# SmartTensors/NMFk.jl

Measured on NVIDIA B200. Metric: nmf_restart_iterations_per_sec, higher is better.
Workload: dtype f32

## Files before the change

nmfk.jl_b200/csrc/kl_tiled.cuh:

```cuda
#pragma once
#include <algorithm>
#include <climits>
#include <cmath>
#include <cstdio>
#include <cstdlib>
#include <type_traits>
#include <chrono>
#include <vector>

#include "kl_resident.cuh"
#include "kl_tiled_args.h"

namespace nmfk {

constexpr int kTiledThreads = 256;
constexpr int kTiledStages = 3;

template <typename TX>
struct TiledCfg {
    static constexpr int TCH = sizeof(TX) == 8 ? 16 : 32;
};


template <typename TX, typename TC, int K, bool HASNAN>
// ... 631 lines not shown
        fprintf(stderr, "\n");
        for (auto e : idle) cudaEventDestroy(e);
        idle.clear();
    }
};

#define NMFK_TRY(call)                      \
    do {                                    \
        cudaError_t e__ = (call);           \
        if (e__ != cudaSuccess) {           \
            err = e__;                      \
            goto done;                      \
        }                                   \
    } while (0)

template <typename TX, typename TC>
cudaError_t solve_tiled_t(const SolveArgs& a, cudaStream_t s, int64_t* launches) {
    const int n = a.n, m = a.m, k = a.k, R = a.R;
    const int kt = tiled_template_k(k);
    if (kt < 0) return cudaErrorInvalidValue;
    cudaError_t err = cudaSuccess;
    int sms = 148;
    {
        int dev = 0;
        cudaGetDevice(&dev);
        cudaDeviceGetAttribute(&sms, cudaDevAttrMultiProcessorCount, dev);
    }
    bool use_tc = false;
    if (std::is_same<TX, float>::value && std::is_same<TC, float>::value && a.tiled_tc && !a.has_nan) {
        TiledPassArgs probe{};
        probe.k = k;
        probe.nown = m;
        probe.D = a.Xt;
        use_tc = tc_pass_supported(probe);
        probe.nown = n;
        probe.D = a.X;
        use_tc = use_tc && tc_pass_supported(probe);
    }
    const bool use_td = std::is_same<TX, double>::value && std::is_same<TC, double>::value && a.tiled_tc && !a.has_nan && k >= 4;
    const int ownper = use_tc ? 128 : (use_td ? tiled_dmma_own() : kTiledThreads);
    const int units = use_tc ? (R + tc_pass_group(k) - 1) / tc_pass_group(k) : R;
    const int nblkH = (m + ownper - 1) / ownper;
    const int nblkW = (n + ownper - 1) / ownper;
    constexpr int TCH = TiledCfg<TX>::TCH;
    const double slice_gain = getenv("NMFK_TILED_SLICE_GAIN") ? atof(getenv("NMFK_TILED_SLICE_GAIN")) : 0.05;
    auto slices = [&](int nblk, int nred) {
        const long long target = (use_tc ? 3ll * tc_pass_ctas_per_sm(k) : (use_td ? 3ll : 4ll)) * sms;
        long long S = (target + (long long)nblk * units - 1) / ((long long)nblk * units);
        const long long smax = std::max(1, nred / ((use_tc ? tc_pass_chunk(k) : (use_td ? tiled_dmma_chunk() : TCH)) * 8));
        if (S > smax) S = smax;
        if (S < 1) S = 1;
        auto eff = [&](long long s_) {
            const long long ctas = (long long)nblk * units * s_;
            return (double)ctas / (double)(((ctas + sms - 1) / sms) * sms);
        };
        long long best = S;
        for (long long s2 = S + 1; s2 <= std::min(smax, S + 3); ++s2)
            if (eff(s2) > eff(best) + slice_gain) best = s2;
        return (int)best;
    };
    const int SH = slices(nblkH, n), SW = slices(nblkW, m);
    const int nblkObj = (n + 127) / 128;
    const bool wobj = a.wref.any();

    const ShardComm* sh = a.shard;
    const bool sharded = sh != nullptr;
    PhaseTimer pt;
    pt.on = getenv("NMFK_TILED_TIMING") != nullptr;
    const auto host_t0 = std::chrono::steady_clock::now();
    auto host_ms = [&]() { return std::chrono::duration<double, std::milli>(std::chrono::steady_clock::now() - host_t0).count(); };
    double host_setup_ms = 0.0;
    const int it_begin_report = 0;
    (void)it_begin_report;
    TC* den = nullptr;
    TC* red = nullptr;
    double* obj2 = nullptr;
    TC* partial = nullptr;
    double* objp = nullptr;
    int* d_active = nullptr;
    double* fin_tot = nullptr;
    int* fin_flag = nullptr;
    void* vimg = nullptr;
    int* h_active = nullptr;
    const char* flag_kernel = use_tc && tc2_pass_enabled(k) ? "tc2_pass_kernel or tc_pass_kernel" : "tc_pass_kernel";
    const char* flag_where = "half-update pass or stop-check objective";
    std::vector<UnitState> hst((size_t)R);
    int it = 0;
    bool any_running = false;
    const size_t psz = std::max((size_t)((SH > 1 || sharded) ? (size_t)SH * R * m * kt : 0),
                                (size_t)(SW > 1 ? (size_t)SW * R * n * kt : 0));
    const size_t redsz = sharded ? (size_t)R * m * kt : 0;
    if (sharded && a.normalize == 2) return cudaErrorNotSupported;
    const int wait_hint = getenv("NMFK_TC_WAIT_HINT_NS") ? atoi(getenv("NMFK_TC_WAIT_HINT_NS")) : ((32 << 16) | 64);
    const int qwait = getenv("NMFK_TC_QWAIT_NS") ? atoi(getenv("NMFK_TC_QWAIT_NS")) : 0;
    auto obj_args = [&](int restore, int sel) {
        TiledPassArgs po{};
        po.D = use_td ? a.Xt : a.X;
        po.U = a.W;
        po.V = a.H;
        po.st = a.st;
        po.u_rstride = (long long)n * k;
        po.v_rstride = (long long)k * m;
        po.su_o = 1;
        po.su_a = n;
        po.sv_t = k;
        po.sv_a = 1;
        po.nown = n;
        po.nred = m;
        po.k = k;
        po.R = R;
        po.S = 1;
        po.nblocks = nblkObj;
        po.lambda = a.lambda;
        po.ktmpl = kt;
        po.obj_partials = objp;
        po.obj_weight = a.weight;
        po.obj_restore = restore;
        po.obj_sel = sel;
        po.wait_hint_ns = wait_hint;
        po.qwait_ns = qwait;
        return po;
    };

    NMFK_TRY(scratch_alloc(&den, ((size_t)R * kTiledMaxK + redsz) * sizeof(TC), s));
    if (sharded) red = den + (size_t)R * kTiledMaxK;
    NMFK_TRY(scratch_alloc(&obj2, (size_t)R * 2 * sizeof(double), s));
    if (psz) NMFK_TRY(scratch_alloc(&partial, psz * sizeof(TC), s));
    NMFK_TRY(scratch_alloc(&objp, (size_t)R * nblkObj * 2 * sizeof(double), s));
    NMFK_TRY(scratch_alloc(&d_active, sizeof(int), s));
    NMFK_TRY(scratch_alloc(&fin_tot, (size_t)R * kTiledMaxK * sizeof(double), s));
    NMFK_TRY(scratch_alloc(&fin_flag, (size_t)R * sizeof(int), s));
    if (use_tc) {
        const size_t vb = std::max(tc2_image_bytes(k, R, n), tc2_image_bytes(k, R, m));
        if (vb) NMFK_TRY(scratch_alloc(&vimg, vb, s));
    }
    h_active = pinned_flags();
    if (h_active == nullptr) NMFK_TRY(cudaErrorMemoryAllocation);
    h_active[0] = h_active[1] = 0;
    h_active[1] = 0;
    NMFK_TRY(cudaMemcpyAsync(hst.data(), a.st, (size_t)R * sizeof(UnitState), cudaMemcpyDeviceToHost, s));
    NMFK_TRY(cudaStreamSynchronize(s));
    for (auto& u : hst)
        if (u.stop == 0 && !u.done) {
            any_running = true;
            it = std::max(it, (int)u.it);
        }
    if (any_running) {
        TiledPassArgs ph{}, pw{};
        ph.D = use_td ? a.X : a.Xt;
        ph.Dstep = a.X;
        ph.U = a.H;
        ph.V = a.W;
        ph.den = den;
        ph.partial = (SH > 1 || sharded) ? partial : nullptr;
        ph.st = a.st;
        ph.ximp = a.ximp;
        ph.u_rstride = (long long)k * m;
        ph.v_rstride = (long long)n * k;
        ph.su_o = k;
        ph.su_a = 1;
        ph.sv_t = 1;
        ph.sv_a = n;
        ph.nown = m;
        ph.nred = n;
        ph.k = k;
        ph.R = R;
        ph.S = SH;
        ph.nblocks = nblkH;
        ph.transposed = 1;
        ph.ldimp = n;
        ph.has_nan = a.has_nan;
        ph.lambda = a.lambda;
        ph.ktmpl = kt;
        ph.vimg = vimg;
        ph.wait_hint_ns = wait_hint;
        ph.qwait_ns = qwait;
        pw = ph;
        pw.D = use_td ? a.Xt : a.X;
        pw.Dstep = a.Xt;
        pw.U = a.W;
        pw.V = a.H;
        pw.partial = SW > 1 ? partial : nullptr;
        pw.u_rstride = (long long)n * k;
        pw.v_rstride = (long long)k * m;
        pw.su_o = 1;
        pw.su_a = n;
        pw.sv_t = k;
        pw.sv_a = 1;
        pw.nown = n;
        pw.nred = m;
        pw.S = SW;
        pw.nblocks = nblkW;
        pw.transposed = 0;

        if (a.has_nan && it > 0) {
            dim3 g((n + 127) / 128, R);
            tiled_impute_kernel<TX, TC><<<g, 128, 0, s>>>((const TX*)a.X, n, m, k, (const TC*)a.W, (const TC*)a.H, a.st,
                                                          (TC*)a.ximp);
            NMFK_TRY(cudaGetLastError());
            ++*launches;
        }
        long long* d_trace = nullptr;
        const char* trace_path = use_tc ? getenv("NMFK_TC_TRACE") : nullptr;
// ... 11 lines not shown
                                                                   d_active);
                NMFK_TRY(cudaGetLastError());
                ++*launches;
                NMFK_TRY(cudaMemcpyAsync(h_active, d_active, sizeof(int), cudaMemcpyDeviceToHost, s));
                pt.mark(s, 10);
                NMFK_TRY(cudaStreamSynchronize(s));
                if (a.prof) a.prof->harvest();
                pt.harvest();
                if (h_active[1] != 0) goto done;
                if (*h_active == 0) break;
                need_guard = false;
                pt.mark(s, -1);
            }
            ++it;
            ph.first_iter = pw.first_iter = (it == 1);
            if (!a.Hfixed) {
                tiled_sums_kernel<TC><<<dim3(k, R), 256, 0, s>>>(a.W, (long long)n * k, 1, n, n, a.st, den);
                NMFK_TRY(cudaGetLastError());
                pt.mark(s, 0);
                NMFK_TRY((timed_tiled_pass<TX, TC>(ph, red, s, use_tc, h_active + 1, use_td, a.prof)));
                pt.mark(s, 1);
                *launches += 2 + (SH > 1 || sharded) + (vimg != nullptr);
                if (d_trace != nullptr) {
                    std::vector<long long> ht(3 * 64 * 8);
                    NMFK_TRY(cudaMemcpyAsync(ht.data(), d_trace, ht.size() * sizeof(long long), cudaMemcpyDeviceToHost, s));
                    NMFK_TRY(cudaStreamSynchronize(s));
                    if (FILE* f = fopen(trace_path, "wb")) {
                        fwrite(ht.data(), sizeof(long long), ht.size(), f);
                        fclose(f);
                    }
                    cudaFree(d_trace);
                    d_trace = nullptr;
                    ph.trace = nullptr;
                }
                if (sharded) {
                    NMFK_TRY(sh->allreduce(sh->comm, den, (size_t)R * kTiledMaxK + redsz, sizeof(TC) == 8 ? 1 : 0, s));
                    pt.mark(s, 2);
                    NMFK_TRY((dispatch_tiled_apply<TX, TC>(ph, red, s)));
                    pt.mark(s, 3);
                    ++*launches;
                }
            }
            if (!a.Wfixed) {
                tiled_sums_kernel<TC><<<dim3(k, R), 256, 0, s>>>(a.H, (long long)k * m, k, 1, m, a.st, den);
                NMFK_TRY(cudaGetLastError());
                pt.mark(s, 4);
                NMFK_TRY((timed_tiled_pass<TX, TC>(pw, nullptr, s, use_tc, h_active + 1, use_td, a.prof)));
                pt.mark(s, 5);
                *launches += 2 + (SW > 1) + (vimg != nullptr);
            }
            if (a.has_nan) {
                dim3 g((n + 127) / 128, R);
                tiled_impute_kernel<TX, TC><<<g, 128, 0, s>>>((const TX*)a.X, n, m, k, (const TC*)a.W, (const TC*)a.H,
                                                              a.st, (TC*)a.ximp);
                NMFK_TRY(cudaGetLastError());
                ++*launches;
            }
            if (it % a.check_every == 0) {
                if (use_tc && !wobj) {
                    NMFK_TRY(launch_tc_objective(obj_args(0, 0), h_active + 1, s));
                } else if (use_td && !wobj) {
                    NMFK_TRY(launch_tiled_dmma_objective(obj_args(0, 0), s));
                } else {
                    dim3 g(nblkObj, R);
                    NMFK_TRY((tiled_objective_smem<TX, TC>(k)));
                    tiled_objective_kernel<TX, TC><<<g, 128, (size_t)k * 128 * sizeof(TC), s>>>(
                        (const TX*)a.X, n, m, k, (const TC*)a.W, (const TC*)a.H, a.st, (TC)a.lambda, 0, 1, a.weight, a.wref, objp);
                }
                NMFK_TRY(cudaGetLastError());
                pt.mark(s, 7);
                tiled_objsum_kernel<<<(R + 127) / 128, 128, 0, s>>>(objp, nblkObj, R, obj2);
                NMFK_TRY(cudaGetLastError());
                ++*launches;
                if (sharded) NMFK_TRY(sh->allreduce(sh->comm, obj2, (size_t)R * 2, 1, s));
                pt.mark(s, 8);
                const bool wide_clamp = (long long)n * k >= (1ll << 18) && !a.Wfixed;
                if (wide_clamp) {
                    const long long nk = (long long)n * k;
                    dim3 g((unsigned)std::min<long long>((nk + 2047) / 2048, 4096), R);
                    tiled_clampW_kernel<TC><<<g, 256, 0, s>>>((TC*)a.W, nk, a.st, obj2, a.tol, (TC)a.eps_clamp);
                    NMFK_TRY(cudaGetLastError());
                    ++*launches;
                }
                TiledCheckArgs c{};
                c.W = a.W;
                c.H = a.H;
                c.st = a.st;
                c.canon = a.canon;
                c.partials = obj2;
                c.n = n;
                c.m = m;
                c.k = k;
                c.nblk = 1;
                c.w_clamped = wide_clamp ? 1 : 0;
                c.it = it;
                c.maxbad = a.maxbad;
                c.stopconv = a.stopconv;
                c.tol = a.tol;
                c.tolOF = a.tolOF;
                c.eps_clamp = a.eps_clamp;
                {
                    const size_t csm = (size_t)(m + k) * sizeof(int);
                    if (csm > 48 * 1024)
                        NMFK_TRY(cudaFuncSetAttribute(tiled_check_kernel<TC>, cudaFuncAttributeMaxDynamicSharedMemorySize, (int)csm));
                    tiled_check_kernel<TC><<<R, 256, csm, s>>>(c);
                }
                NMFK_TRY(cudaGetLastError());
                pt.mark(s, 9);
                *launches += 2;
                need_guard = true;
            }
            if (it >= a.maxiter || (a.iter_limit > 0 && it >= a.iter_limit)) need_guard = true;
        }
    }
    {
        pt.mark(s, -1);
        flag_kernel = "tc_pass_kernel";
        flag_where = "post-run objective";
        if (use_tc && !wobj) {
            NMFK_TRY(launch_tc_objective(obj_args(1, 1), h_active + 1, s));
        } else if (use_td && !wobj) {
            NMFK_TRY(launch_tiled_dmma_objective(obj_args(1, 1), s));
        } else {
            dim3 g(nblkObj, R);
            NMFK_TRY((tiled_objective_smem<TX, TC>(k)));
            tiled_objective_kernel<TX, TC><<<g, 128, (size_t)k * 128 * sizeof(TC), s>>>(
                (const TX*)a.X, n, m, k, (const TC*)a.W, (const TC*)a.H, a.st, (TC)a.lambda, 1, 0, a.weight, a.wref, objp);
        }
        NMFK_TRY(cudaGetLastError());
        if (sharded) {
            tiled_objsum_kernel<<<(R + 127) / 128, 128, 0, s>>>(objp, nblkObj, R, obj2);
            NMFK_TRY(cudaGetLastError());
            NMFK_TRY(sh->allreduce(sh->comm, obj2, (size_t)R * 2, 1, s));
            ++*launches;
        }
        const bool wide_finish = a.normalize == 1 && (long long)n * k >= (1ll << 18);
        if (wide_finish) NMFK_TRY(cudaMemsetAsync(fin_flag, 0, (size_t)R * sizeof(int), s));
        tiled_finish_kernel<TC><<<R, 256, 0, s>>>(a.W, a.H, a.st, sharded ? obj2 : objp, n, m, k, sharded ? 1 : nblkObj,
                                                  a.normalize, wide_finish ? fin_tot : nullptr, wide_finish ? fin_flag : nullptr);
        NMFK_TRY(cudaGetLastError());
        if (wide_finish) {
            const long long nk = (long long)n * k;
            dim3 g((unsigned)std::min<long long>((nk + 2047) / 2048, 1024), R);
            tiled_scaleW_kernel<TC><<<g, 256, 0, s>>>((TC*)a.W, n, k, fin_tot, fin_flag);
            NMFK_TRY(cudaGetLastError());
            ++*launches;
        }
        *launches += 2;
        pt.mark(s, 11);
        NMFK_TRY(cudaStreamSynchronize(s));
        if (a.prof) a.prof->harvest();
        pt.harvest();
        if (pt.on) fprintf(stderr, "[nmfk timing] host wall clock: set-up %.1f ms, whole solve %.1f ms\n", host_setup_ms, host_ms());
        pt.report(it, sharded ? sh->rank : 0);
    }
done:
    if (h_active && h_active[1] != 0) err = solve_timeout(a, err, flag_kernel, flag_where, h_active[1]);
    scratch_free(den, s);
    scratch_free(partial, s);
    scratch_free(objp, s);
    scratch_free(obj2, s);
    scratch_free(d_active, s);
    scratch_free(fin_tot, s);
    scratch_free(fin_flag, s);
    scratch_free(vimg, s);
    return err;
}

}
```

nmfk.jl_b200/csrc/kl_tiled_args.h:

```cpp
#pragma once
#include "nmfk_internal.h"

namespace nmfk {

struct TiledPassArgs {
    const void* D;
    void* U;
    const void* V;
    const void* den;
    void* partial;
    const UnitState* st;
    const void* ximp;
    long long u_rstride, v_rstride;
    long long su_o, su_a, sv_t, sv_a;
    int nown, nred, k, R, S, nblocks;
    int transposed;
    int ldimp;
    int has_nan, first_iter;
    double lambda;
    double* obj_partials;
    double obj_weight;
    int obj_restore;
    int obj_sel;
    int wait_hint_ns;
    int qwait_ns;
    long long* trace;
    int ktmpl;
    const void* Dstep;
    void* vimg;
};

bool tc_pass_supported(const TiledPassArgs& a);
int tc_pass_group(int k);
int tc_pass_ctas_per_sm(int k);
int tc_pass_chunk(int k);
cudaError_t launch_tc_pass(const TiledPassArgs& a, int* d_errflag, cudaStream_t s);
bool tc2_pass_enabled(int k);
cudaError_t launch_tc2_pass(const TiledPassArgs& a, int* d_errflag, cudaStream_t s);
size_t tc2_image_bytes(int k, int R, int nred);
void tc2_pass_prepare();
cudaError_t launch_tc_objective(const TiledPassArgs& a, int* d_errflag, cudaStream_t s);

int tiled_dmma_own();
int tiled_dmma_chunk();
cudaError_t launch_tiled_dmma_pass(const TiledPassArgs& a, cudaStream_t s);
cudaError_t launch_tiled_dmma_objective(const TiledPassArgs& a, cudaStream_t s);

}
```

nmfk.jl_b200/csrc/kl_tiled_tc.cu:

```cuda
#include <algorithm>

#include "kl_tiled_args.h"
#include "tc_ptx.cuh"
#include "tc_stage.cuh"

namespace nmfk {
namespace {

constexpr int TC_M = 128;

template <int K8, int N2>
struct TcCfg {
    static constexpr int TS = 64;
    static constexpr int NXS = K8 <= 32 ? 3 : 2;
    static constexpr int NRAW = K8 <= 32 ? 4 : 2;
    static constexpr int NVB = K8 <= 16 ? 4 : (K8 <= 32 ? 3 : 2);
    static constexpr int RPAD = K8 > 24 ? 0 : 4;
    static constexpr int QW = TS / 4;
    static constexpr int SW = 4;
    static constexpr int QW0 = 2 + SW;
    static constexpr int THREADS = (QW0 + QW) * 32;
    static constexpr int TCOLS = 512;
    static constexpr int NCS = QW / 4;
    static constexpr int NST = N2 == 16 ? 2 : 1;
// ... 437 lines not shown
            tc::named_bar_sync(2, TC_QWARPS * 32);
            if (grp == 1)
#pragma unroll
                for (int c = 0; c < NC2; ++c) xch[c * 256 + slot] = acc[0][c];
            tc::named_bar_sync(2, TC_QWARPS * 32);
            if (grp == 0)
#pragma unroll
                for (int c = 0; c < NC2; ++c) acc[0][c] += xch[c * 256 + slot];
        }
#pragma unroll
        for (int i = 0; i < SL; ++i) {
            const int b = 2 * i + grp;
            if (b < nreal && valid) {
                const int r = s_act[b];
                if (a.partial == nullptr) {
                    float* U = Ug + (long long)r * a.u_rstride;
                    const float* den = static_cast<const float*>(a.den) + (long long)r * kTiledMaxK;
#pragma unroll
                    for (int c = 0; c < NC2; ++c) {
                        const int col = hh * NC2 + c;
                        if (col < k) {
                            const long long idx = (long long)o * a.su_o + (long long)col * a.su_a;
                            U[idx] = (U[idx] * acc[i][c]) / den[col];
                        }
                    }
                } else {
                    float* dst = static_cast<float*>(a.partial) + (((long long)slice * a.R + r) * a.nown + o) * a.ktmpl;
#pragma unroll
                    for (int c = 0; c < NC2; ++c) {
                        const int col = hh * NC2 + c;
                        if (col < a.ktmpl) dst[col] = acc[i][c];
                    }
                }
            }
        }
        }
        __syncwarp();
    }
    tc::tc_fence_before_sync();
    __syncthreads();
    if (warp == 0) tc::tmem_dealloc<C::TCOLS>(tbase);
}

template <int K8, int N2, bool OBJ>
cudaError_t launch_tc(const TiledPassArgs& a, int* d_errflag, cudaStream_t s) {
    using C = TcCfg<K8, N2>;
    const int ngroups = (a.R + C::RB - 1) / C::RB;
    const long long grid = (long long)a.S * a.nblocks * ngroups;
    if (grid > 2147483647ll) return cudaErrorInvalidValue;
    cudaError_t e = cudaFuncSetAttribute(tc_pass_kernel<K8, N2, OBJ>, cudaFuncAttributeMaxDynamicSharedMemorySize, (int)C::SMEM);
    if (e != cudaSuccess) return e;
    tc_pass_kernel<K8, N2, OBJ><<<(unsigned)grid, C::THREADS, C::SMEM, s>>>(a, d_errflag);
    return cudaGetLastError();
}

}

int tc_pass_group(int k) {
    if (k <= 8) return TcCfg<8, 16>::RB;
    if (k <= 16) return TcCfg<16, 16>::RB;
    if (k <= 24) return TcCfg<24, 32>::RB;
    if (k <= 32) return TcCfg<32, 32>::RB;
    if (k <= 48) return TcCfg<48, 64>::RB;
    return TcCfg<64, 64>::RB;
}
int tc_pass_ctas_per_sm(int) { return 1; }
int tc_pass_chunk(int) { return 64; }

bool tc_pass_supported(const TiledPassArgs& a) {
    return !a.has_nan && a.k >= 1 && a.k <= kTiledMaxK && (a.nown % 4) == 0 && (reinterpret_cast<uintptr_t>(a.D) % 16) == 0;
}

cudaError_t launch_tc_pass(const TiledPassArgs& a, int* d_errflag, cudaStream_t s) {
    if (tc2_pass_enabled(a.k)) return launch_tc2_pass(a, d_errflag, s);
    if (a.k <= 8) return launch_tc<8, 16, false>(a, d_errflag, s);
    if (a.k <= 16) return launch_tc<16, 16, false>(a, d_errflag, s);
    if (a.k <= 24) return launch_tc<24, 32, false>(a, d_errflag, s);
    if (a.k <= 32) return launch_tc<32, 32, false>(a, d_errflag, s);
    if (a.k <= 48) return launch_tc<48, 64, false>(a, d_errflag, s);
    return launch_tc<64, 64, false>(a, d_errflag, s);
}

cudaError_t launch_tc_objective(const TiledPassArgs& a, int* d_errflag, cudaStream_t s) {
    if (a.k <= 8) return launch_tc<8, 16, true>(a, d_errflag, s);
    if (a.k <= 16) return launch_tc<16, 16, true>(a, d_errflag, s);
    if (a.k <= 24) return launch_tc<24, 32, true>(a, d_errflag, s);
    if (a.k <= 32) return launch_tc<32, 32, true>(a, d_errflag, s);
    if (a.k <= 48) return launch_tc<48, 64, true>(a, d_errflag, s);
    return launch_tc<64, 64, true>(a, d_errflag, s);
}

}
```

nmfk.jl_b200/csrc/kl_tiled_tc2.cu:

```cuda
#include <algorithm>
#include <cstdlib>
#include <mutex>

#include "kl_tiled_args.h"
#include "tc_ptx.cuh"
#include "tc_stage.cuh"
#include "tma.cuh"

namespace nmfk {
namespace {

constexpr int T2_M = 128;

template <int K8>
struct Tc2Cfg {
    static constexpr int N2 = 16;
    static constexpr int TS = 64;
    static constexpr int NXS = 3;
    static constexpr int NVB = 6;
    static constexpr int QW = TS / 4;
    static constexpr int QW0 = 2;
    static constexpr int LW = QW0 + QW;
    static constexpr int THREADS = (LW + 1) * 32;
    static constexpr int TCOLS = 512;
    static constexpr int RB = 4;
    static constexpr int ACOLS = 2 * N2;
    static constexpr int PBASE = 0, QBASE = 2 * TS, ABASE = QBASE + 2 * 2 * TS, UBASE = ABASE + 2 * ACOLS;
    static constexpr int PERB = K8;
    static_assert(UBASE + RB * PERB <= TCOLS, "tensor memory");
    static constexpr uint32_t U1_BYTES = T2_M * K8 * 4;
    static constexpr uint32_t SBO1 = (K8 / 4) * 128;
    static constexpr uint32_t SBO2 = (TS / 4) * 128;
    static constexpr uint32_t B1_BYTES = TS * K8 * 4;
    static constexpr uint32_t B2_BYTES = N2 * TS * 4;
    static constexpr uint32_t V_BYTES = 2 * B1_BYTES + 2 * B2_BYTES;
    static constexpr uint32_t X_BYTES = TS * T2_M * 4;
    static constexpr int XBOX = 32;
    static constexpr size_t SMEM = (size_t)NXS * X_BYTES + (size_t)NVB * V_BYTES + (size_t)RB * U1_BYTES + 32 * 8 + 64;
    static_assert(SMEM <= 232448, "shared memory budget of one CTA");
};

__device__ __forceinline__ unsigned long long pack2f(float lo, float hi) {
    unsigned long long v;
    asm("mov.b64 %0, {%1, %2};" : "=l"(v) : "f"(lo), "f"(hi));
    return v;
}
__device__ __forceinline__ float rcp_approx(float p) {
    float r;
    asm("rcp.approx.ftz.f32 %0, %1;" : "=f"(r) : "f"(p));
    return r;
}

template <int K8>
__global__ void __launch_bounds__(256) tc2_images_kernel(const TiledPassArgs a, int chunks) {
    using C = Tc2Cfg<K8>;
    const int c = blockIdx.x, r = blockIdx.y;
    if (a.st[r].stop != 0) return;
    const float* V = static_cast<const float*>(a.V) + (long long)r * a.v_rstride;
    float4* img = reinterpret_cast<float4*>(static_cast<unsigned char*>(a.vimg) + ((size_t)r * chunks + c) * C::V_BYTES);
    const int t0 = c * C::TS;
    auto val = [&](int t, int col) {
        return (t0 + t < a.nred && col < a.k) ? V[(long long)(t0 + t) * a.sv_t + (long long)col * a.sv_a] : 0.f;
    };
    constexpr int NAB = K8 / 4, NTB = C::TS / 4;
    constexpr int NA = C::TS * NAB, NB = C::N2 * NTB;
    for (int it = threadIdx.x; it < NA + NB; it += blockDim.x) {
        float v[4];
        int hi, lo;
        if (it < NA) {
            const int t = (it & 7) + 8 * (it / (8 * NAB)), ab = (it >> 3) % NAB;
#pragma unroll
            for (int j = 0; j < 4; ++j) v[j] = val(t, ab * 4 + j);
            hi = it;
            lo = it + C::B1_BYTES / 16;
        } else {
            const int ib = it - NA;
            const int col = (ib & 7) + 8 * (ib / (8 * NTB)), tb = (ib >> 3) % NTB;
#pragma unroll
            for (int i = 0; i < 4; ++i) v[i] = val(tb * 4 + i, col);
            hi = 2 * C::B1_BYTES / 16 + ib;
            lo = hi + C::B2_BYTES / 16;
        }
        float h[4], l[4];
#pragma unroll
        for (int j = 0; j < 4; ++j) {
            h[j] = __uint_as_float(__float_as_uint(v[j]) & 0xffffe000u);
            l[j] = v[j] - h[j];
        }
        img[hi] = make_float4(h[0], h[1], h[2], h[3]);
        img[lo] = make_float4(l[0], l[1], l[2], l[3]);
    }
}

template <int K8>
__global__ void __launch_bounds__((Tc2Cfg<K8>::THREADS), 1) tc2_pass_kernel(const TiledPassArgs a, const __grid_constant__ CUtensorMap mX,
                                                                            int* errflag) {
    using C = Tc2Cfg<K8>;
    constexpr int NXS = C::NXS, NVB = C::NVB, TS = C::TS, QWARPS = C::QW, QW0 = C::QW0;
    constexpr int RB = C::RB, N2 = C::N2;
    extern __shared__ __align__(1024) unsigned char smem[];
    float* Xs = reinterpret_cast<float*>(smem);
    unsigned char* Vs = smem + (size_t)NXS * C::X_BYTES;
    unsigned char* Us = Vs + (size_t)NVB * C::V_BYTES;
    uint64_t* bars = reinterpret_cast<uint64_t*>(Us + (size_t)RB * C::U1_BYTES);
    uint64_t* x_full = bars;
    uint64_t* x_empty = x_full + NXS;
    uint64_t* v_full = x_empty + NXS;
    uint64_t* v_empty = v_full + NVB;
    uint64_t* p_full = v_empty + NVB;
    uint64_t* p_empty = p_full + 2;
    uint64_t* q_full = p_empty + 2;
    uint64_t* a_full = q_full + 2;
    uint32_t* tmem_slot = reinterpret_cast<uint32_t*>(bars + 32);
    int* s_act = reinterpret_cast<int*>(tmem_slot + 1);

    const int tid = threadIdx.x, warp = tid >> 5, lane = tid & 31;
    long long* const trc = (a.trace != nullptr && blockIdx.x == 0) ? a.trace : nullptr;
    const int ngroups = (a.R + RB - 1) / RB;
    const int g = blockIdx.x % ngroups;
    const int rest = blockIdx.x / ngroups;
    const int ob = rest % a.nblocks;
    const int slice = rest / a.nblocks;
    const int o0 = ob * T2_M;
    const int k = a.k;
    const int chunks_all = (a.nred + TS - 1) / TS;
    const int t_begin = (int)(((long long)chunks_all * slice) / a.S) * TS;
    const int t_end = min(a.nred, (int)(((long long)chunks_all * (slice + 1)) / a.S) * TS);
    const int nchunks = (t_end - t_begin + TS - 1) / TS;

    if (tid == 0) {
        int nact = 0;
        for (int b = 0; b < RB; ++b) {
            const int r = g * RB + b;
            if (r >= a.R) continue;
            if (a.st[r].stop == 0) s_act[nact++] = r;
        }
        s_act[RB] = nact;
        if (nact & 1) s_act[nact] = s_act[0];
    }
    __syncthreads();
    const int nreal = s_act[RB];
    const int nact = nreal + (nreal & 1);
    if (nreal == 0 || nchunks <= 0) return;
    const int total = nchunks * nact;

    if (warp == 0) tc::tmem_alloc<C::TCOLS>(tmem_slot);
    if (tid == 32) {
        for (int i = 0; i < NXS; ++i) {
// ... 234 lines not shown
                            float q = xv[j] * rcp_approx(__uint_as_float(p[jj]));
                            q = (jh + half * 16 + jj < cnt) ? q : 0.f;
                            const uint32_t h = __float_as_uint(q) & 0xffffe000u;
                            lo[j] = __float_as_uint(q - __uint_as_float(h));
                            p[jj] = h;
                        }
                    }
                    if (prev_slot >= 0) {
                        if (half == 0) {
                            if (warp == QW0) TC_STAMP(0, u, 5);
                            tc::mbar_wait_h(0u, &a_full[grp], (uint32_t)(((u - 2) >> 1) & 1), errflag, 44);
                            tc::tc_fence_after_sync();
                            if (warp == QW0) TC_STAMP(0, u, 6);
                        } else {
                            tc::tmem_wait_ld();
                            drain_add(prev_slot);
                        }
                        drain_load(half);
                    }
                    tc::tmem_st16(qcol + half * 16, p);
                    tc::tmem_st16(qcol + TS + half * 16, lo);
                    if (half == 0 && warp == QW0) TC_STAMP(0, u, 7);
                }
                if (prev_slot >= 0) {
                    tc::tmem_wait_ld();
                    drain_add(prev_slot);
                }
                if (warp == QW0) TC_STAMP(0, u, 3);
                tc::tmem_wait_st();
                tc::tc_fence_before_sync();
                __syncwarp();
                if (lane == 0) tc::mbar_arrive(&q_full[grp]);
                if (warp == QW0) TC_STAMP(0, u, 4);
                prev_slot = b >> 1;
            }
            __syncwarp();
            if (lane == 0) tc::mbar_arrive(&x_empty[s]);
        }
        {
            const int ulast = (nchunks - 1) * nact + (nact - 2 + grp);
            tc::mbar_wait_h(0u, &a_full[grp], (uint32_t)((ulast >> 1) & 1), errflag, 43);
            tc::tc_fence_after_sync();
#pragma unroll
            for (int part = 0; part < 2; ++part) {
                drain_load(part);
                tc::tmem_wait_ld();
                drain_add(prev_slot);
            }
        }
#pragma unroll
        for (int i = 0; i < SL; ++i) {
            const int b = 2 * i + grp;
            if (b < nreal && valid) {
                const int r = s_act[b];
                if (a.partial == nullptr) {
                    float* U = Ug + (long long)r * a.u_rstride;
                    const float* den = static_cast<const float*>(a.den) + (long long)r * kTiledMaxK;
#pragma unroll
                    for (int c = 0; c < NC2; ++c) {
                        const int col = hh * NC2 + c;
                        if (col < k) {
                            const long long idx = (long long)o * a.su_o + (long long)col * a.su_a;
                            U[idx] = (U[idx] * acc[i][c]) / den[col];
                        }
                    }
                } else {
                    float* dst = static_cast<float*>(a.partial) + (((long long)slice * a.R + r) * a.nown + o) * a.ktmpl;
#pragma unroll
                    for (int c = 0; c < NC2; ++c) {
                        const int col = hh * NC2 + c;
                        if (col < a.ktmpl) dst[col] = acc[i][c];
                    }
                }
            }
        }
        __syncwarp();
    }
    tc::tc_fence_before_sync();
    __syncthreads();
    if (warp == 0) tc::tmem_dealloc<C::TCOLS>(tbase);
}

template <int K8>
cudaError_t launch2(const TiledPassArgs& a, int* d_errflag, cudaStream_t s) {
    using C = Tc2Cfg<K8>;
    const int ngroups = (a.R + C::RB - 1) / C::RB;
    const long long grid = (long long)a.S * a.nblocks * ngroups;
    const int chunks = (a.nred + C::TS - 1) / C::TS;
    if (grid > 2147483647ll || a.vimg == nullptr || a.R > 65535) return cudaErrorInvalidValue;
    cudaError_t e = cudaFuncSetAttribute(tc2_pass_kernel<K8>, cudaFuncAttributeMaxDynamicSharedMemorySize, (int)C::SMEM);
    if (e != cudaSuccess) return e;
    struct Cached {
        const void* base;
        int nown, nred;
        CUtensorMap map;
    };
    static std::mutex mu;
    static Cached cache[4];
    static int next = 0;
    CUtensorMap mX;
    {
        std::lock_guard<std::mutex> lock(mu);
        int hit = -1;
        for (int i = 0; i < 4; ++i)
            if (cache[i].base == a.Dstep && cache[i].nown == a.nown && cache[i].nred == a.nred) hit = i;
        if (hit < 0) {
            hit = next;
            next = (next + 1) % 4;
            cache[hit].base = nullptr;
            if (!tma_make_map_f32(&cache[hit].map, a.Dstep, a.nred, a.nown, a.nred, C::XBOX, T2_M, CU_TENSOR_MAP_SWIZZLE_128B))
                return cudaErrorNotSupported;
            cache[hit].base = a.Dstep;
            cache[hit].nown = a.nown;
            cache[hit].nred = a.nred;
        }
        mX = cache[hit].map;
    }
    tc2_images_kernel<K8><<<dim3((unsigned)chunks, (unsigned)a.R), 256, 0, s>>>(a, chunks);
    e = cudaGetLastError();
    if (e != cudaSuccess) return e;
    tc2_pass_kernel<K8><<<(unsigned)grid, C::THREADS, C::SMEM, s>>>(a, mX, d_errflag);
    return cudaGetLastError();
}

}

bool tc2_pass_enabled(int k) {
    static const int gen = [] {
        const char* e = std::getenv("NMFK_TC_GEN");
        return e ? std::atoi(e) : 2;
    }();
    return gen >= 2 && k <= 16 && tma_encode_fn() != nullptr;
}

size_t tc2_image_bytes(int k, int R, int nred) {
    const size_t per = k <= 8 ? Tc2Cfg<8>::V_BYTES : Tc2Cfg<16>::V_BYTES;
    constexpr int TS = Tc2Cfg<16>::TS;
    return tc2_pass_enabled(k) ? (size_t)R * (size_t)((nred + TS - 1) / TS) * per : 0;
}

void tc2_pass_prepare() {
    static bool done = false;
    if (done) return;
    done = true;
    CUtensorMap m;
    float* dummy = nullptr;
    if (cudaMalloc(&dummy, 1 << 20) == cudaSuccess) {
        (void)tma_make_map_f32(&m, dummy, 512, 512, 512, 32, T2_M, CU_TENSOR_MAP_SWIZZLE_128B);
        cudaFree(dummy);
    }
    cudaFuncAttributes fa;
    cudaFuncGetAttributes(&fa, tc2_pass_kernel<8>);
    cudaFuncGetAttributes(&fa, tc2_pass_kernel<16>);
    cudaFuncSetAttribute(tc2_pass_kernel<8>, cudaFuncAttributeMaxDynamicSharedMemorySize, (int)Tc2Cfg<8>::SMEM);
    cudaFuncSetAttribute(tc2_pass_kernel<16>, cudaFuncAttributeMaxDynamicSharedMemorySize, (int)Tc2Cfg<16>::SMEM);
}

cudaError_t launch_tc2_pass(const TiledPassArgs& a, int* d_errflag, cudaStream_t s) {
    if (a.k <= 8) return launch2<8>(a, d_errflag, s);
    return launch2<16>(a, d_errflag, s);
}

}
```

Baseline: 7466.

## Add TMA/tcgen05 pipelined objective kernel for tc2 path

Adds a new warp-specialized objective kernel that uses TMA loads of X, bulk copies of precomputed V images, and split-TF32 tensor-memory MMAs to compute the Frobenius objective, replacing the older tc objective when tc2 is enabled. It reuses the tc2 image kernel in an objective-only mode and factors the tensor map cache into a shared helper. The aim is faster stop-check objective evaluations. The cost is an extra image-building launch per objective and more complex barrier pipelines.

```diff
diff --git a/nmfk.jl_b200/csrc/kl_tiled.cuh b/nmfk.jl_b200/csrc/kl_tiled.cuh
--- a/nmfk.jl_b200/csrc/kl_tiled.cuh
+++ b/nmfk.jl_b200/csrc/kl_tiled.cuh
@@ -737,7 +737,8 @@
     int* fin_flag = nullptr;
     void* vimg = nullptr;
     int* h_active = nullptr;
-    const char* flag_kernel = use_tc && tc2_pass_enabled(k) ? "tc2_pass_kernel or tc_pass_kernel" : "tc_pass_kernel";
+    const bool tc2 = use_tc && tc2_pass_enabled(k);
+    const char* flag_kernel = tc2 ? "tc2_pass_kernel or tc2_objective_kernel" : "tc_pass_kernel";
     const char* flag_where = "half-update pass or stop-check objective";
     std::vector<UnitState> hst((size_t)R);
     int it = 0;
@@ -774,6 +775,8 @@
         po.obj_sel = sel;
         po.wait_hint_ns = wait_hint;
         po.qwait_ns = qwait;
+        po.Dstep = a.Xt;
+        po.vimg = vimg;
         return po;
     };
 
@@ -951,6 +954,7 @@
                     NMFK_TRY(cudaGetLastError());
                     ++*launches;
                 }
+                if (tc2 && !wobj) ++*launches;
                 TiledCheckArgs c{};
                 c.W = a.W;
                 c.H = a.H;
@@ -984,10 +988,11 @@
     }
     {
         pt.mark(s, -1);
-        flag_kernel = "tc_pass_kernel";
+        flag_kernel = tc2 ? "tc2_objective_kernel" : "tc_pass_kernel";
         flag_where = "post-run objective";
         if (use_tc && !wobj) {
             NMFK_TRY(launch_tc_objective(obj_args(1, 1), h_active + 1, s));
+            if (tc2) ++*launches;
         } else if (use_td && !wobj) {
             NMFK_TRY(launch_tiled_dmma_objective(obj_args(1, 1), s));
         } else {
diff --git a/nmfk.jl_b200/csrc/kl_tiled_args.h b/nmfk.jl_b200/csrc/kl_tiled_args.h
--- a/nmfk.jl_b200/csrc/kl_tiled_args.h
+++ b/nmfk.jl_b200/csrc/kl_tiled_args.h
@@ -40,6 +40,7 @@
 size_t tc2_image_bytes(int k, int R, int nred);
 void tc2_pass_prepare();
 cudaError_t launch_tc_objective(const TiledPassArgs& a, int* d_errflag, cudaStream_t s);
+cudaError_t launch_tc2_objective(const TiledPassArgs& a, int* d_errflag, cudaStream_t s);
 
 int tiled_dmma_own();
 int tiled_dmma_chunk();
diff --git a/nmfk.jl_b200/csrc/kl_tiled_tc.cu b/nmfk.jl_b200/csrc/kl_tiled_tc.cu
--- a/nmfk.jl_b200/csrc/kl_tiled_tc.cu
+++ b/nmfk.jl_b200/csrc/kl_tiled_tc.cu
@@ -543,6 +543,7 @@
 }
 
 cudaError_t launch_tc_objective(const TiledPassArgs& a, int* d_errflag, cudaStream_t s) {
+    if (tc2_pass_enabled(a.k) && a.vimg != nullptr && a.Dstep != nullptr) return launch_tc2_objective(a, d_errflag, s);
     if (a.k <= 8) return launch_tc<8, 16, true>(a, d_errflag, s);
     if (a.k <= 16) return launch_tc<16, 16, true>(a, d_errflag, s);
     if (a.k <= 24) return launch_tc<24, 32, true>(a, d_errflag, s);
diff --git a/nmfk.jl_b200/csrc/kl_tiled_tc2.cu b/nmfk.jl_b200/csrc/kl_tiled_tc2.cu
--- a/nmfk.jl_b200/csrc/kl_tiled_tc2.cu
+++ b/nmfk.jl_b200/csrc/kl_tiled_tc2.cu
@@ -51,19 +51,26 @@
     return r;
 }
 
-template <int K8>
+template <bool OBJ>
+__device__ __forceinline__ bool tc2_takes(const TiledPassArgs& a, int r) {
+    const bool stopped = a.st[r].stop != 0;
+    return (OBJ && a.obj_sel == 1) ? (stopped && a.st[r].done == 0) : !stopped;
+}
+
+template <int K8, bool OBJ>
 __global__ void __launch_bounds__(256) tc2_images_kernel(const TiledPassArgs a, int chunks) {
     using C = Tc2Cfg<K8>;
+    constexpr uint32_t IMG = OBJ ? 2 * C::B1_BYTES : C::V_BYTES;
     const int c = blockIdx.x, r = blockIdx.y;
-    if (a.st[r].stop != 0) return;
+    if (!tc2_takes<OBJ>(a, r)) return;
     const float* V = static_cast<const float*>(a.V) + (long long)r * a.v_rstride;
-    float4* img = reinterpret_cast<float4*>(static_cast<unsigned char*>(a.vimg) + ((size_t)r * chunks + c) * C::V_BYTES);
+    float4* img = reinterpret_cast<float4*>(static_cast<unsigned char*>(a.vimg) + ((size_t)r * chunks + c) * IMG);
     const int t0 = c * C::TS;
     auto val = [&](int t, int col) {
         return (t0 + t < a.nred && col < a.k) ? V[(long long)(t0 + t) * a.sv_t + (long long)col * a.sv_a] : 0.f;
     };
     constexpr int NAB = K8 / 4, NTB = C::TS / 4;
-    constexpr int NA = C::TS * NAB, NB = C::N2 * NTB;
+    constexpr int NA = C::TS * NAB, NB = OBJ ? 0 : C::N2 * NTB;
     for (int it = threadIdx.x; it < NA + NB; it += blockDim.x) {
         float v[4];
         int hi, lo;
@@ -464,6 +471,319 @@
 }
 
 template <int K8>
+struct Tc2ObjCfg {
+    using C = Tc2Cfg<K8>;
+    static constexpr int TS = C::TS, RB = C::RB;
+    static constexpr int NXS = 3;
+    static constexpr int NVB = 8;
+    static constexpr int NP = 6;
+    static constexpr int SW0 = 2;
+    static constexpr int NSW = TS / 4;
+    static constexpr int THREADS = (SW0 + NSW) * 32;
+    static constexpr int TCOLS = 512;
+    static constexpr int PBASE = 0, UBASE = NP * TS;
+    static_assert(UBASE + RB * C::PERB <= TCOLS, "tensor memory");
+    static constexpr uint32_t IMG = 2 * C::B1_BYTES;
+    static constexpr int NBARS = 2 * (NXS + NVB + NP);
+    static constexpr size_t SMEM = (size_t)NXS * C::X_BYTES + (size_t)NVB * IMG + (size_t)RB * C::U1_BYTES + NBARS * 8 + 64;
+    static_assert(SMEM <= 232448, "shared memory budget of one CTA");
+};
+
+template <int K8>
+__global__ void __launch_bounds__((Tc2ObjCfg<K8>::THREADS), 1) tc2_objective_kernel(const TiledPassArgs a,
+                                                                                    const __grid_constant__ CUtensorMap mX, int* errflag) {
+    using C = Tc2Cfg<K8>;
+    using O = Tc2ObjCfg<K8>;
+    constexpr int NXS = O::NXS, NVB = O::NVB, NP = O::NP, TS = O::TS, RB = O::RB, SW0 = O::SW0, NSW = O::NSW;
+    extern __shared__ __align__(1024) unsigned char smem[];
+    float* Xs = reinterpret_cast<float*>(smem);
+    unsigned char* Vs = smem + (size_t)NXS * C::X_BYTES;
+    unsigned char* Us = Vs + (size_t)NVB * O::IMG;
+    uint64_t* bars = reinterpret_cast<uint64_t*>(Us + (size_t)RB * C::U1_BYTES);
+    uint64_t* x_full = bars;
+    uint64_t* x_empty = x_full + NXS;
+    uint64_t* v_full = x_empty + NXS;
+    uint64_t* v_empty = v_full + NVB;
+    uint64_t* p_full = v_empty + NVB;
+    uint64_t* p_empty = p_full + NP;
+    uint32_t* tmem_slot = reinterpret_cast<uint32_t*>(bars + O::NBARS);
+    int* s_act = reinterpret_cast<int*>(tmem_slot + 1);
+
+    const int tid = threadIdx.x, warp = tid >> 5, lane = tid & 31;
+    const int ngroups = (a.R + RB - 1) / RB;
+    const int g = blockIdx.x % ngroups;
+    const int ob = blockIdx.x / ngroups;
+    const int o0 = ob * T2_M;
+    const int k = a.k;
+    const int nchunks = (a.nred + TS - 1) / TS;
+
+    if (tid == 0) {
+        int nact = 0;
+        for (int b = 0; b < RB; ++b) {
+            const int r = g * RB + b;
+            if (r < a.R && tc2_takes<true>(a, r)) s_act[nact++] = r;
+        }
+        s_act[RB] = nact;
+    }
+    __syncthreads();
+    const int nact = s_act[RB];
+    if (nact == 0 || nchunks <= 0) return;
+    const int total = nchunks * nact;
+
+    if (warp == 0) tc::tmem_alloc<O::TCOLS>(tmem_slot);
+    if (tid == 32) {
+        for (int i = 0; i < NXS; ++i) {
+            tc::mbar_init(&x_full[i], 1);
+            tc::mbar_init(&x_empty[i], NSW);
+        }
+        for (int i = 0; i < NVB; ++i) {
+            tc::mbar_init(&v_full[i], 1);
+            tc::mbar_init(&v_empty[i], 1);
+        }
+        for (int i = 0; i < NP; ++i) {
+            tc::mbar_init(&p_full[i], 1);
+            tc::mbar_init(&p_empty[i], NSW);
+        }
+        tc::mbar_fence_init();
+    }
+    if (tid == 0) tma_prefetch_map(&mX);
+
+    tc::fence_async_smem();
+    tc::tc_fence_before_sync();
+    __syncthreads();
+    tc::tc_fence_after_sync();
+    const uint32_t tbase = *tmem_slot;
+
+    if (warp >= SW0) {
+        const int lq = warp & 3, cs = (warp - SW0) >> 2;
+        const int ol = lq * 32 + lane;
+        const int o = o0 + ol;
+        const bool valid = o < a.nown;
+        const uint32_t lane_base = tbase + ((uint32_t)(lq * 32) << 16);
+        if (cs < nact) {
+            const float* U = static_cast<const float*>(a.U) + (long long)s_act[cs] * a.u_rstride;
+            const uint32_t col = O::UBASE + cs * C::PERB;
+            unsigned char* img = Us + (size_t)cs * C::U1_BYTES + (ol & 7) * 16 + (ol >> 3) * C::SBO1;
+#pragma unroll
+            for (int c0 = 0; c0 < K8; c0 += 8) {
+                uint32_t hi[8];
+                float lo[8];
+#pragma unroll
+                for (int c = 0; c < 8; ++c) {
+                    const float u = !valid ? 1.f : (c0 + c < k ? U[(long long)o * a.su_o + (long long)(c0 + c) * a.su_a] : 0.f);
+                    hi[c] = __float_as_uint(u) & 0xffffe000u;
+                    lo[c] = u - __uint_as_float(hi[c]);
+                }
+                tc::tmem_st8(lane_base + col + c0, hi);
+                *reinterpret_cast<float4*>(img + (c0 / 4) * TC_LBO) = make_float4(lo[0], lo[1], lo[2], lo[3]);
+                *reinterpret_cast<float4*>(img + (c0 / 4 + 1) * TC_LBO) = make_float4(lo[4], lo[5], lo[6], lo[7]);
+            }
+        }
+        tc::tmem_wait_st();
+    }
+    tc::fence_async_smem();
+    tc::tc_fence_before_sync();
+    __syncthreads();
+    tc::tc_fence_after_sync();
+
+    if (warp == 0) {
+        constexpr uint32_t idP = tc::idesc_tf32(T2_M, TS, 0);
+        const uint64_t d1 = tc::smem_desc(tc::smem_u32(Vs), TC_LBO, C::SBO1);
+        const uint64_t du = tc::smem_desc(tc::smem_u32(Us), TC_LBO, C::SBO1);
+        constexpr uint64_t KSTEP = (2 * TC_LBO) >> 4;
+        int b = 0, vb = 0, pt = 0;
+        for (int u = 0; u < total; ++u) {
+            if (u >= NP) tc::mbar_wait_h(0u, &p_empty[pt], (uint32_t)((u / NP - 1) & 1), errflag, 51);
+            tc::mbar_wait_h(0u, &v_full[vb], (uint32_t)((u / NVB) & 1), errflag, 50);
+            tc::tc_fence_after_sync();
+            const uint32_t d = tbase + O::PBASE + (uint32_t)pt * TS;
+            const uint32_t uh = tbase + O::UBASE + b * C::PERB;
+            const uint64_t al = du + (uint64_t)((b * C::U1_BYTES) >> 4);
+            const uint64_t bh = d1 + (uint64_t)((vb * O::IMG) >> 4), bl = bh + (C::B1_BYTES >> 4);
+            if (tc::elect_one()) {
+#pragma unroll
+                for (int ks = 0; ks < K8 / 8; ++ks) {
+                    tc::mma_tf32_ss(d, al + ks * KSTEP, bh + ks * KSTEP, idP, ks > 0);
+                    tc::mma_tf32_ts(d, uh + ks * 8, bl + ks * KSTEP, idP, 1);
+                    tc::mma_tf32_ts(d, uh + ks * 8, bh + ks * KSTEP, idP, 1);
+                }
+                tc::mma_commit(&p_full[pt]);
+                tc::mma_commit(&v_empty[vb]);
+            }
+            __syncwarp();
+            b = b + 1 == nact ? 0 : b + 1;
+            vb = vb + 1 == NVB ? 0 : vb + 1;
+            pt = pt + 1 == NP ? 0 : pt + 1;
+        }
+        __syncwarp();
+    } else if (warp == 1) {
+        auto load_x = [&](int c, int s) {
+            if (tc::elect_one()) {
+                tc::mbar_arrive_expect_tx(&x_full[s], C::X_BYTES);
+                tma_load_2d(Xs + (size_t)s * TS * T2_M, &mX, c * TS, o0, &x_full[s]);
+                tma_load_2d(Xs + (size_t)s * TS * T2_M + C::XBOX * T2_M, &mX, c * TS + C::XBOX, o0, &x_full[s]);
+            }
+            __syncwarp();
+        };
+        for (int c = 0; c < NXS && c < nchunks; ++c) load_x(c, c);
+        const unsigned char* vimg = static_cast<const unsigned char*>(a.vimg);
+        int c = 0, b = 0, s = 0;
+        int vb = 0, vround = 0;
+        for (int w = 0; w < total; ++w) {
+            if (b == 0 && c >= NXS) {
+                tc::mbar_wait_h(0u, &x_empty[s], (uint32_t)((c / NXS - 1) & 1), errflag, 52);
+                load_x(c, s);
+            }
+            if (vround > 0) tc::mbar_wait_h(0u, &v_empty[vb], (uint32_t)((vround - 1) & 1), errflag, 53);
+            if (tc::elect_one()) {
+                tc::mbar_arrive_expect_tx(&v_full[vb], O::IMG);
+                tc::bulk_g2s(Vs + (size_t)vb * O::IMG, vimg + ((size_t)s_act[b] * nchunks + c) * O::IMG, O::IMG, &v_full[vb]);
+            }
+            __syncwarp();
+            if (++vb == NVB) vb = 0, ++vround;
+            if (++b == nact) {
+                b = 0;
+                ++c;
+                s = s + 1 == NXS ? 0 : s + 1;
+            }
+        }
+        __syncwarp();
+    } else {
+        const int lq = warp & 3, cs = (warp - SW0) >> 2;
+        const int o_loc = lq * 32 + lane;
+        const bool valid = o0 + o_loc < a.nown;
+        const uint32_t lane_base = tbase + ((uint32_t)(lq * 32) << 16);
+        const int j0 = cs * 16;
+        const uint32_t xrow = (uint32_t)((cs >> 1) * C::XBOX * T2_M + o_loc * C::XBOX) * 4;
+        const uint32_t xsw = ((tc::smem_u32(Xs) + xrow) >> 7) & 7;
+        const uint32_t xp0 = (uint32_t)(cs & 1) * 4;
+        double sacc[RB];
+#pragma unroll
+        for (int b = 0; b < RB; ++b) sacc[b] = 0.0;
+        const float lambda = (float)a.lambda;
+        const bool restore = a.obj_restore != 0;
+        auto pull = [&](int u, int t, uint32_t(&p)[16]) {
+            tc::mbar_wait_h(0u, &p_full[t], (uint32_t)((u / NP) & 1), errflag, 55);
+            tc::tc_fence_after_sync();
+            tc::tmem_ld16(lane_base + O::PBASE + (uint32_t)t * TS + j0, p);
+        };
+        auto pulled = [&](int t) {
+            tc::tmem_wait_ld();
+            tc::tc_fence_before_sync();
+            __syncwarp();
+            if (lane == 0) tc::mbar_arrive(&p_empty[t]);
+        };
+        int c = 0, b = 0, pt = 0;
+        int cnt = TS;
+        bool full = false;
+        float xv[16];
+        auto step = [&](int u, const uint32_t(&p)[16], uint32_t(&pn)[16]) {
+            if (b == 0) {
+                const int s = c % NXS;
+                cnt = min(TS, a.nred - c * TS);
+                tc::mbar_wait_h(0u, &x_full[s], (uint32_t)((c / NXS) & 1), errflag, 54);
+                const unsigned char* xs = reinterpret_cast<const unsigned char*>(Xs + (size_t)s * TS * T2_M) + xrow;
+#pragma unroll
+                for (int i = 0; i < 4; ++i) {
+                    const float4 x4 = *reinterpret_cast<const float4*>(xs + (((xp0 + i) ^ xsw) << 4));
+                    xv[4 * i] = x4.x, xv[4 * i + 1] = x4.y, xv[4 * i + 2] = x4.z, xv[4 * i + 3] = x4.w;
+                }
+#pragma unroll
+                for (int j = 0; j < 16; ++j)
+                    if (restore && xv[j] == lambda) xv[j] = 0.f;
+                __syncwarp();
+                if (lane == 0) tc::mbar_arrive(&x_empty[s]);
+                full = valid && cnt == TS;
+            }
+            const int tn = pt + 1 == NP ? 0 : pt + 1;
+            const bool more = u + 1 < total;
+            if (more) pull(u + 1, tn, pn);
+            float su = 0.f;
+            if (full) {
+#pragma unroll
+                for (int j = 0; j < 16; j += 2) {
+                    unsigned long long e2;
+                    asm("sub.rn.f32x2 %0, %1, %2;"
+                        : "=l"(e2)
+                        : "l"(pack2f(xv[j], xv[j + 1])), "l"(pack2f(__uint_as_float(p[j]), __uint_as_float(p[j + 1]))));
+                    const float e0 = __uint_as_float((uint32_t)e2), e1 = __uint_as_float((uint32_t)(e2 >> 32));
+                    su = fmaf(e0, e0, su);
+                    su = fmaf(e1, e1, su);
+                }
+            } else {
+#pragma unroll
+                for (int j = 0; j < 16; ++j) {
+                    float e = xv[j] - __uint_as_float(p[j]);
+                    e = (valid && j0 + j < cnt) ? e : 0.f;
+                    su = fmaf(e, e, su);
+                }
+            }
+#pragma unroll
+            for (int bb = 0; bb < RB; ++bb)
+                if (bb == b) sacc[bb] += (double)su;
+            if (more) pulled(tn);
+            pt = tn;
+            if (++b == nact) b = 0, ++c;
+        };
+        uint32_t pa[16], pb[16];
+        pull(0, 0, pa);
+        pulled(0);
+        for (int u = 0; u < total; u += 2) {
+            step(u, pa, pb);
+            if (u + 1 < total) step(u + 1, pb, pa);
+        }
+        double* red = reinterpret_cast<double*>(Xs);
+        __syncwarp();
+        tc::named_bar_sync(2, NSW * 32);
+#pragma unroll
+        for (int b = 0; b < RB; ++b) {
+            double v = sacc[b];
+#pragma unroll
+            for (int off = 16; off > 0; off >>= 1) v += __shfl_xor_sync(0xffffffffu, v, off);
+            if (lane == 0) red[b * NSW + (warp - SW0)] = v;
+        }
+        tc::named_bar_sync(2, NSW * 32);
+        if (warp == SW0 && lane < nact) {
+            double t = 0.0;
+            for (int w = 0; w < NSW; ++w) t += red[lane * NSW + w];
+            double* dst = a.obj_partials + ((long long)s_act[lane] * a.nblocks + ob) * 2;
+            dst[0] = t * a.obj_weight * a.obj_weight;
+            dst[1] = t;
+        }
+    }
+    tc::tc_fence_before_sync();
+    __syncthreads();
+    if (warp == 0) tc::tmem_dealloc<O::TCOLS>(tbase);
+}
+
+bool x_map(const TiledPassArgs& a, CUtensorMap* out) {
+    struct Cached {
+        const void* base;
+        int nown, nred;
+        CUtensorMap map;
+    };
+    static std::mutex mu;
+    static Cached cache[4];
+    static int next = 0;
+    std::lock_guard<std::mutex> lock(mu);
+    int hit = -1;
+    for (int i = 0; i < 4; ++i)
+        if (cache[i].base == a.Dstep && cache[i].nown == a.nown && cache[i].nred == a.nred) hit = i;
+    if (hit < 0) {
+        hit = next;
+        next = (next + 1) % 4;
+        cache[hit].base = nullptr;
+        if (!tma_make_map_f32(&cache[hit].map, a.Dstep, a.nred, a.nown, a.nred, Tc2Cfg<16>::XBOX, T2_M, CU_TENSOR_MAP_SWIZZLE_128B))
+            return false;
+        cache[hit].base = a.Dstep;
+        cache[hit].nown = a.nown;
+        cache[hit].nred = a.nred;
+    }
+    *out = cache[hit].map;
+    return true;
+}
+
+template <int K8>
 cudaError_t launch2(const TiledPassArgs& a, int* d_errflag, cudaStream_t s) {
     using C = Tc2Cfg<K8>;
     const int ngroups = (a.R + C::RB - 1) / C::RB;
@@ -472,36 +792,30 @@
     if (grid > 2147483647ll || a.vimg == nullptr || a.R > 65535) return cudaErrorInvalidValue;
     cudaError_t e = cudaFuncSetAttribute(tc2_pass_kernel<K8>, cudaFuncAttributeMaxDynamicSharedMemorySize, (int)C::SMEM);
     if (e != cudaSuccess) return e;
-    struct Cached {
-        const void* base;
-        int nown, nred;
-        CUtensorMap map;
-    };
-    static std::mutex mu;
-    static Cached cache[4];
-    static int next = 0;
     CUtensorMap mX;
-    {
-        std::lock_guard<std::mutex> lock(mu);
-        int hit = -1;
-        for (int i = 0; i < 4; ++i)
-            if (cache[i].base == a.Dstep && cache[i].nown == a.nown && cache[i].nred == a.nred) hit = i;
-        if (hit < 0) {
-            hit = next;
-            next = (next + 1) % 4;
-            cache[hit].base = nullptr;
-            if (!tma_make_map_f32(&cache[hit].map, a.Dstep, a.nred, a.nown, a.nred, C::XBOX, T2_M, CU_TENSOR_MAP_SWIZZLE_128B))
-                return cudaErrorNotSupported;
-            cache[hit].base = a.Dstep;
-            cache[hit].nown = a.nown;
-            cache[hit].nred = a.nred;
-        }
-        mX = cache[hit].map;
-    }
-    tc2_images_kernel<K8><<<dim3((unsigned)chunks, (unsigned)a.R), 256, 0, s>>>(a, chunks);
+    if (!x_map(a, &mX)) return cudaErrorNotSupported;
+    tc2_images_kernel<K8, false><<<dim3((unsigned)chunks, (unsigned)a.R), 256, 0, s>>>(a, chunks);
     e = cudaGetLastError();
     if (e != cudaSuccess) return e;
     tc2_pass_kernel<K8><<<(unsigned)grid, C::THREADS, C::SMEM, s>>>(a, mX, d_errflag);
+    return cudaGetLastError();
+}
+
+template <int K8>
+cudaError_t launch2_objective(const TiledPassArgs& a, int* d_errflag, cudaStream_t s) {
+    using O = Tc2ObjCfg<K8>;
+    const int ngroups = (a.R + O::RB - 1) / O::RB;
+    const long long grid = (long long)a.nblocks * ngroups;
+    const int chunks = (a.nred + O::TS - 1) / O::TS;
+    if (a.S != 1 || grid > 2147483647ll || a.vimg == nullptr || a.R > 65535) return cudaErrorInvalidValue;
+    cudaError_t e = cudaFuncSetAttribute(tc2_objective_kernel<K8>, cudaFuncAttributeMaxDynamicSharedMemorySize, (int)O::SMEM);
+    if (e != cudaSuccess) return e;
+    CUtensorMap mX;
+    if (!x_map(a, &mX)) return cudaErrorNotSupported;
+    tc2_images_kernel<K8, true><<<dim3((unsigned)chunks, (unsigned)a.R), 256, 0, s>>>(a, chunks);
+    e = cudaGetLastError();
+    if (e != cudaSuccess) return e;
+    tc2_objective_kernel<K8><<<(unsigned)grid, O::THREADS, O::SMEM, s>>>(a, mX, d_errflag);
     return cudaGetLastError();
 }
 
@@ -536,6 +850,10 @@
     cudaFuncGetAttributes(&fa, tc2_pass_kernel<16>);
     cudaFuncSetAttribute(tc2_pass_kernel<8>, cudaFuncAttributeMaxDynamicSharedMemorySize, (int)Tc2Cfg<8>::SMEM);
     cudaFuncSetAttribute(tc2_pass_kernel<16>, cudaFuncAttributeMaxDynamicSharedMemorySize, (int)Tc2Cfg<16>::SMEM);
+    cudaFuncGetAttributes(&fa, tc2_objective_kernel<8>);
+    cudaFuncGetAttributes(&fa, tc2_objective_kernel<16>);
+    cudaFuncSetAttribute(tc2_objective_kernel<8>, cudaFuncAttributeMaxDynamicSharedMemorySize, (int)Tc2ObjCfg<8>::SMEM);
+    cudaFuncSetAttribute(tc2_objective_kernel<16>, cudaFuncAttributeMaxDynamicSharedMemorySize, (int)Tc2ObjCfg<16>::SMEM);
 }
 
 cudaError_t launch_tc2_pass(const TiledPassArgs& a, int* d_errflag, cudaStream_t s) {
@@ -543,4 +861,9 @@
     return launch2<16>(a, d_errflag, s);
 }
 
-}
+cudaError_t launch_tc2_objective(const TiledPassArgs& a, int* d_errflag, cudaStream_t s) {
+    if (a.k <= 8) return launch2_objective<8>(a, d_errflag, s);
+    return launch2_objective<16>(a, d_errflag, s);
+}
+
+}
```

After: 7701, median of 6. 1.03x the previous value.
